# SamsungLabs/fcaf3d

Hardware: AMD Instinct MI355X
Metric: scenes/sec fwd+bwd, ScanNet 100k-pt 2cm voxels, 1/2/4/8 MI355X (higher is better)
Workload: dtype f32

## Files before the change

### fcaf3d_amd/csrc/conv.hip

```cpp
#include "fc_common.h"
#include "../../include/fcaf3d_hip.h"
#ifdef FC_TRACE
__device__ unsigned long long* g_trace_buf_lds;
__device__ int g_trace_cap_lds;
extern "C" int fc_debug_trace_lds(unsigned long long* buf, int cap) {
  FC_HIP(hipMemcpyToSymbol(HIP_SYMBOL(g_trace_buf_lds), &buf, sizeof(buf)));
  FC_HIP(hipMemcpyToSymbol(HIP_SYMBOL(g_trace_cap_lds), &cap, sizeof(cap)));
  return FC_OK;
}
#define TR_BUF g_trace_buf_lds
#define TR_CAP g_trace_cap_lds
#endif
#include "fc_trace.h"

typedef float f32x16 __attribute__((ext_vector_type(16)));
typedef float f32x2 __attribute__((ext_vector_type(2)));
typedef float f32x4 __attribute__((ext_vector_type(4)));

__device__ __attribute__((aligned(16))) float g_zero_row[64];

__device__ int g_fc_prio;
extern "C" int fc_debug_set_prio(int mode) {
  FC_HIP(hipMemcpyToSymbol(HIP_SYMBOL(g_fc_prio), &mode, sizeof(mode)));
  return FC_OK;
}

static int g_bf16_fast = 0;
extern "C" int fc_set_bf16_fast(int on) {
  g_bf16_fast = on ? 1 : 0;
  return FC_OK;
}

static int g_split_mode = 2;
static inline int split_mode() { return g_bf16_fast ? 0 : g_split_mode; }
extern "C" int fc_set_split_mode(int mode) {
  if (mode != 0 && mode != 2) return FC_EINVAL;
  g_split_mode = mode;
  return FC_OK;
}
extern "C" int fc_get_split_mode(void) { return split_mode(); }
static int g_h3r = 1;
extern "C" int fc_debug_set_h3r(int mode) {
  if (mode < 0 || mode > 2) return FC_EINVAL;
  g_h3r = mode;
  return FC_OK;
}

#include <mutex>
#include "conv_tile.h"
#include "conv_f32.h"
#include "wgrad_f32.h"
#include "conv_stem.h"
#include "conv_x6.h"
#include "wgrad_x6.h"
#include "conv_h3r.h"
#include "conv_route.h"
static inline RouteEnv route_env() { return {split_mode(), g_bf16_fast, g_h3r}; }

__global__ __launch_bounds__(256) void k_amax(const f32x4* __restrict__ x, int64_t n4, const float* __restrict__ tail, int ntail,
                                              unsigned* __restrict__ slot) {
  __shared__ unsigned wm[4];
  __shared__ int last_s;
  unsigned m = 0u;
  const int64_t stride = (int64_t)gridDim.x * 256;
  for (int64_t i = (int64_t)blockIdx.x * 256 + threadIdx.x; i < n4; i += 4 * stride) {
    f32x4 v[4];
#pragma unroll
    for (int q = 0; q < 4; ++q) v[q] = i + q * stride < n4 ? x[i + q * stride] : f32x4{0.f, 0.f, 0.f, 0.f};
#pragma unroll
    for (int q = 0; q < 4; ++q)
#pragma unroll
      for (int j = 0; j < 4; ++j) { const unsigned u = __float_as_uint(v[q][j]) & 0x7fffffffu; m = (u > m && u < 0x7f800000u) ? u : m; }
  }
  if (blockIdx.x == 0 && (int)threadIdx.x < ntail) { const unsigned u = __float_as_uint(tail[threadIdx.x]) & 0x7fffffffu; m = (u > m && u < 0x7f800000u) ? u : m; }
#pragma unroll
  for (int off = 32; off > 0; off >>= 1) { const unsigned o = (unsigned)__shfl_xor((int)m, off, 64); m = o > m ? o : m; }
  if ((threadIdx.x & 63) == 0) wm[threadIdx.x >> 6] = m;
  __syncthreads();
  if (threadIdx.x == 0) {
    unsigned b = wm[0];
    for (int w = 1; w < 4; ++w) b = wm[w] > b ? wm[w] : b;
    if (b > __hip_atomic_load(&slot[1], __ATOMIC_RELAXED, __HIP_MEMORY_SCOPE_AGENT)) atomicMax(&slot[1], b);
    __threadfence();
    last_s = atomicAdd(&slot[2], 1u) == gridDim.x - 1;
    if (last_s) {
      __threadfence();
      slot[0] = atomicExch(&slot[1], 0u);
      slot[2] = 0u;
    }
  }
}

constexpr int AMAX_RING = 2048;
static unsigned* g_amax_ring[16] = {};
static unsigned g_amax_next[16] = {};
static std::mutex g_amax_ring_mu;
static int amax_ring_slot(unsigned** slot) {
  int dev = 0;
  FC_HIP(hipGetDevice(&dev));
  if (dev < 0 || dev >= 16) return FC_EINVAL;
  std::lock_guard<std::mutex> lock(g_amax_ring_mu);
  if (!g_amax_ring[dev]) {
    FC_HIP(hipMalloc((void**)&g_amax_ring[dev], (size_t)AMAX_RING * FC_AMAX_SLOT_BYTES));
    FC_HIP(hipMemset(g_amax_ring[dev], 0, (size_t)AMAX_RING * FC_AMAX_SLOT_BYTES));
  }
  const unsigned i = __atomic_fetch_add(&g_amax_next[dev], 1u, __ATOMIC_RELAXED) % AMAX_RING;
  *slot = g_amax_ring[dev] + (size_t)i * (FC_AMAX_SLOT_BYTES / 4);
  return FC_OK;
}
static int amax_launch(const float* x, int64_t n, unsigned* slot, hipStream_t stream) {
// ... 145 lines not shown
#pragma unroll
      for (int u = 0; u < 9; ++u) {
        j[u] = k0 + u < K ? pos[(int64_t)(k0 + u) * n_out + o] : -1;
        j2[u] = (two && k0 + u < K) ? pos[(int64_t)(k0 + u) * n_out + o2] : -1;
      }
      f32x4 v[9], v2[9];
#pragma unroll
      for (int u = 0; u < 9; ++u) {
        const float* src = j[u] >= 0 ? part + ((int64_t)(k0 + u) * n_out + j[u]) * Cout + c : g_zero_row + lane * 4;
        const float* src2 = j2[u] >= 0 ? part + ((int64_t)(k0 + u) * n_out + j2[u]) * Cout + c : g_zero_row + lane * 4;
        v[u] = *reinterpret_cast<const f32x4*>(src);
        v2[u] = *reinterpret_cast<const f32x4*>(src2);
      }
#pragma unroll
      for (int u = 0; u < 9; ++u) {
        if (j[u] >= 0) a += v[u];
        if (j2[u] >= 0) b += v2[u];
      }
    }
    *reinterpret_cast<f32x4*>(out + o * Cout + c) = a;
    stat_accumulate(p, epi, a, o * Cout + c, a1, a2);
    if (two) {
      *reinterpret_cast<f32x4*>(out + o2 * Cout + c) = b;
      stat_accumulate(p, epi, b, o2 * Cout + c, a1, a2);
    }
  }
  stat_block_reduce(a1, a2, epi.stats, Cout, sm);
}

static_assert(STEM_CIN == 3 && STEM_COUT == 64 && BK == 32, "conv_route.h spells these shapes out");

struct ConvArgs {
  const float *in, *W; const int *nbr, *out_index, *cnt; float* dst;
  int64_t n_rows; int K, Cin, Cout; X6Epi epi; hipStream_t stream;
};
#define FC_LAUNCH(...) __VA_ARGS__<<<grid, 256, 0, a.stream>>>(a.in, a.W, a.nbr, a.out_index, a.cnt, a.dst, a.n_rows, a.K, a.Cin, a.Cout)
#define FC_LAUNCH_EPI(...) __VA_ARGS__<<<grid, 256, 0, a.stream>>>(a.in, a.W, a.nbr, a.out_index, a.cnt, a.dst, a.n_rows, a.K, a.Cin, a.Cout, a.epi)

template <int BM, int BN, int WM>
static void launch_conv_fp32(const ConvRoute& r, const ConvArgs& a, dim3 grid) {
#define FC_LAUNCH_MFMA(KERNEL)                                                                                              \
  do { if (r.wsrc == FC_WSRC_FP32_T) FC_LAUNCH(KERNEL<BM, BN, 32, true, WM, true>); else if (a.nbr) FC_LAUNCH(KERNEL<BM, BN, 32, true, WM>); \
       else FC_LAUNCH(KERNEL<BM, BN, 32, false, WM>); } while (0)
  if (r.family == FC_FAM_MFMA) FC_LAUNCH_MFMA(k_conv_mfma);
  if constexpr (BM >= 128) {
    if (r.family == FC_FAM_MFMA_P) FC_LAUNCH_MFMA(k_conv_mfma_p);
    if (r.family == FC_FAM_GLDS) { if (a.nbr) FC_LAUNCH(k_conv_glds<BM, BN, true, WM>); else FC_LAUNCH(k_conv_glds<BM, BN, false, WM>); }
  }
#undef FC_LAUNCH_MFMA
}

template <int BM, int BN, int WM>
static void launch_conv_x6(const ConvRoute& r, const ConvArgs& a, dim3 grid) {
  if (r.family == FC_FAM_H3R) {
    if constexpr (BM == 128) {
      if (r.buf) FC_LAUNCH_EPI(k_conv_h3r<BN, true, true>);
      else if (a.nbr) FC_LAUNCH_EPI(k_conv_h3r<BN, true, false>);
      else FC_LAUNCH_EPI(k_conv_h3r<BN, false, false>);
    }
  } else if (r.wsrc == FC_WSRC_FP32_T) FC_LAUNCH_EPI(k_conv_x6<BM, BN, true, WM, 1>);
  else if (r.wsrc == FC_WSRC_FP32) { if (a.nbr) FC_LAUNCH_EPI(k_conv_x6<BM, BN, true, WM, 0>); else FC_LAUNCH_EPI(k_conv_x6<BM, BN, false, WM, 0>); }
  else if (r.mode == FC_MODE_BF16 || r.buf) {
    if constexpr (BM == 128) {
      if (r.mode == FC_MODE_BF16) { if (a.nbr) FC_LAUNCH_EPI(k_conv_x6<128, BN, true, 2, 2, 1>); else FC_LAUNCH_EPI(k_conv_x6<128, BN, false, 2, 2, 1>); }
      else if (r.mode == FC_MODE_H3) FC_LAUNCH_EPI(k_conv_x6<128, BN, true, 2, 2, 2, true>);
      else FC_LAUNCH_EPI(k_conv_x6<128, BN, true, 2, 2, 0, true>);
    }
  } else if (r.mode == FC_MODE_H3) { if (a.nbr) FC_LAUNCH_EPI(k_conv_x6<BM, BN, true, WM, 2, 2>); else FC_LAUNCH_EPI(k_conv_x6<BM, BN, false, WM, 2, 2>); }
  else { if (a.nbr) FC_LAUNCH_EPI(k_conv_x6<BM, BN, true, WM, 2>); else FC_LAUNCH_EPI(k_conv_x6<BM, BN, false, WM, 2>); }
}

static int launch_conv(const ConvRoute& r, const ConvArgs& a) {
  const dim3 grid(r.grid[0], r.grid[1], r.grid[2]);
  if (r.family == FC_FAM_STEM) {
    const size_t smem = (size_t)(STEM_ROWS * STEM_FWD_LDA + 96 * 64) * sizeof(float);
    k_stem_fwd<<<(unsigned)fc_cdiv(a.n_rows, STEM_ROWS), 256, smem, a.stream>>>(a.in, a.W, a.nbr, a.dst, nullptr, a.n_rows, a.K);
  } else if (r.family == FC_FAM_FMA) {
    k_conv_fma<<<(unsigned)fc_cdiv(a.n_rows * a.Cout, 256), 256, 0, a.stream>>>(a.in, a.W, a.nbr, a.dst, a.n_rows, a.K, a.Cin, a.Cout, r.wsrc == FC_WSRC_FP32_T ? 1 : 0);
  } else {
#define FC_TILE(BM, BN, WM) do { if (r.family >= FC_FAM_X6) launch_conv_x6<BM, BN, WM>(r, a, grid); else launch_conv_fp32<BM, BN, WM>(r, a, grid); } while (0)
    if (r.bm == 256) FC_TILE(256, 64, 4);
    else if (r.bm == 128 && r.bn == 128) FC_TILE(128, 128, 2);
    else if (r.bm == 128) FC_TILE(128, 64, 2);
    else if (r.bn == 128) launch_conv_fp32<64, 128, 2>(r, a, grid);
    else launch_conv_fp32<64, 64, 2>(r, a, grid);
#undef FC_TILE
  }
  FC_CHECK_LAUNCH();
  return FC_OK;
}
#undef FC_LAUNCH
#undef FC_LAUNCH_EPI

extern "C" {

int fc_conv_fwd_route(int64_t n_in, int64_t n_out, int K, int Cin, int Cout, int flags, int table_kind, int64_t live_tiles, int* out) {
  if (!out || n_in < 0 || n_out < 0 || K < 1 || Cin < 1 || Cout < 1) return FC_EINVAL;
  const ConvRoute r = conv_route({n_in, n_out, K, Cin, Cout}, flags, table_kind, live_tiles, route_env());
  const int f[16] = {r.family, r.bm, r.bn, r.wm, r.S, r.wsrc, r.mode, r.buf, r.epi, (int)r.grid[0], (int)r.grid[1], (int)r.grid[2]};
  for (int i = 0; i < 16; ++i) out[i] = f[i];
  return r.family == FC_FAM_INVALID ? FC_EINVAL : FC_OK;
}

int64_t fc_conv_fwd_ws_bytes(int64_t n_out, int K, int Cin, int Cout, int flags) {
  const ConvRoute r = conv_route({n_out, n_out, K, Cin, Cout}, flags, FC_TABLE_DENSE, 0, route_env());
  return r.S > 1 ? (int64_t)r.S * n_out * Cout * (int64_t)sizeof(float) : 0;
}

int64_t fc_conv_fwd_pairs_ws_bytes(int64_t n_out, int K, int Cout) {
  return (int64_t)K * n_out * Cout * (int64_t)sizeof(float);
}

int64_t fc_conv_stats_blocks(int64_t n_out, int K, int Cin, int Cout, int flags, int pairs) {
  if (n_out < 1) return 0;
  const ConvRoute r = conv_route({n_out, n_out, K, Cin, Cout}, flags, pairs ? FC_TABLE_PAIRS : FC_TABLE_DENSE, 0, route_env());
  if (r.epi == FC_EPI_NONE) return 0;
  return r.epi == FC_EPI_SUM ? fc_cdiv(n_out, fc_stat_rb(n_out)) : fc_cdiv(n_out, r.bm);
}

static int conv_impl(const float* in, const float* W, const int* nbr, const int* out_index, const int* cnt, const int* pos, float* out,
                     int64_t n_in, int64_t n_out, int K, int Cin, int Cout, int64_t live_tiles, int flags, void* ws, int64_t ws_bytes,
                     hipStream_t stream, const X6Epi* epi) {
  AmaxHintScope hint_scope;
  if (n_in < 0 || n_out < 0 || K < 1 || Cin < 1 || Cout < 1) return FC_EINVAL;
  if (n_out == 0 && !cnt) return epi ? FC_EINVAL : FC_OK;
  if (out_index && !nbr) return FC_EINVAL;
  const int table = cnt ? FC_TABLE_PAIRS : out_index ? FC_TABLE_SORTED : nbr ? FC_TABLE_DENSE : FC_TABLE_NONE;
  const ConvRoute r = conv_route({n_in, n_out, K, Cin, Cout}, flags, table | (epi ? FC_TABLE_STATS : 0), live_tiles, route_env());
  if (r.family == FC_FAM_INVALID) return FC_EINVAL;
  if (n_out == 0) return FC_OK;
  ConvArgs a = {in, W, nbr, out_index, cnt, out, n_out, K, Cin, Cout, {}, stream};
  if (r.family == FC_FAM_STEM || r.family == FC_FAM_FMA) return launch_conv(r, a);
  const bool parts = cnt || r.S > 1;
  if (parts && ws_bytes < (int64_t)r.S * n_out * Cout * (int64_t)sizeof(float)) return FC_EWS;
  if (parts) a.dst = (float*)ws;
  if (epi && r.epi == FC_EPI_KERNEL) a.epi = *epi;
  int rc = FC_OK;
  if (r.mode == FC_MODE_H3) rc = operand_amax(in, n_in * (int64_t)Cin, 0, stream, &a.epi.amax_in);
  if (rc == FC_OK) rc = launch_conv(r, a);
  if (rc != FC_OK || !parts) return rc;
  const int rb = fc_stat_rb(n_out);
  const dim3 sgrid((unsigned)fc_cdiv(n_out, rb), Cout / 64);
  if (cnt && epi) k_sum_pairs_stats<<<sgrid, 256, 0, stream>>>(a.dst, pos, out, n_out, K, Cout, rb, *epi);
  else if (cnt) k_sum_pairs<<<(unsigned)fc_cdiv(n_out * (Cout / 4), 256), 256, 0, stream>>>(a.dst, pos, out, n_out, K, Cout);
  else if (epi) k_sum_parts_stats<<<sgrid, 256, 0, stream>>>(a.dst, out, n_out, Cout, r.S, rb, *epi);
  else k_sum_parts<<<(unsigned)fc_cdiv(n_out * Cout / 4, 256), 256, 0, stream>>>(a.dst, out, n_out * Cout / 4, r.S);
  FC_CHECK_LAUNCH();
  return FC_OK;
}

static int conv_pairs_impl(const float* in, const float* W, const int* pair_in, const int* pair_cnt, const int* pair_pos, float* out,
                           int64_t n_in, int64_t n_out, int K, int Cin, int Cout, int64_t live_tiles, int flags, void* ws,
// ... 323 lines not shown
```

### fcaf3d_amd/csrc/conv_route.h

```cpp
#ifndef FC_CONV_ROUTE_H
#define FC_CONV_ROUTE_H
#include "fc_common.h"
#include "../../include/fcaf3d_hip.h"

struct RouteEnv { int split_mode, bf16_fast, h3r; };
struct ConvShape { int64_t n_in, n_out; int K, Cin, Cout; };

struct ConvRoute {
  int family;
  int bm, bn, wm;
  int S;
  int wsrc, mode, buf, epi;
  unsigned grid[3];
};
struct WgradRoute {
  int family;
  int bm, bn, ko, bkr;
  int table, mode, S;
  int64_t rps;
  int wbuf;
  unsigned grid_y;
};

static inline int flag_bm(int flags) { return (flags >> FC_CONV_BM_SHIFT) & FC_CONV_TILE_MASK; }
static inline int flag_bn(int flags) { return (flags >> FC_CONV_BN_SHIFT) & FC_CONV_TILE_MASK; }
static inline int flag_s(int flags) { return (flags >> FC_CONV_S_SHIFT) & FC_CONV_S_MASK; }
static inline bool below_2gb(uint64_t bytes) { return bytes < (1ull << 31) - 4096u; }

static inline bool stem_shape(int K, int Cin, int Cout, int flags) { return !(flags & FC_CONV_FMA) && Cin == 3 && Cout == 64 && K <= 27; }

static inline int offset_split(int64_t tiles, int K) {
  if (K <= 1 || tiles >= 384) return 1;
  return (int)(1024 / tiles < K ? 1024 / tiles : K);
}

static inline ConvRoute conv_route(const ConvShape& s, int flags, int table, int64_t live_tiles, const RouteEnv& env) {
  const bool stats = (table & FC_TABLE_STATS) != 0;
  table &= ~FC_TABLE_STATS;
  const bool pairs = table == FC_TABLE_PAIRS, gather = table != FC_TABLE_NONE, split = (flags & FC_CONV_SPLIT) != 0;
  const bool image = split && (flags & FC_CONV_IMAGE);
  const bool wt = (flags & FC_CONV_WT) && !image;
  const int64_t n = s.n_out > 0 ? s.n_out : 1;
  const int K = s.K, Cin = s.Cin, Cout = s.Cout;
  ConvRoute r = {};
  r.family = FC_FAM_INVALID;
  r.wsrc = image ? FC_WSRC_IMAGE : wt ? FC_WSRC_FP32_T : FC_WSRC_FP32;
  if (!gather && (K != 1 || s.n_in != s.n_out)) return r;
  if ((flags & FC_CONV_WT) && !gather) return r;
  const bool mfma = Cin % 32 == 0 && Cout % 64 == 0 && (pairs || (!(flags & FC_CONV_FMA) && K <= 32));
  if (pairs && !mfma) return r;
  if (stats && !(mfma && split)) return r;
  r.bn = (Cout % 128 == 0) ? 128 : 64;
  if (pairs) {
    if (flag_bn(flags) == 1) r.bn = 64;
    r.bm = 128;
    r.S = K;
  } else {
    r.bm = (n > 64 && fc_cdiv(n, 128) * (Cout / r.bn) >= 4) ? 128 : 64;
    if (Cout == 64 && fc_cdiv(n, 256) >= 1024 && !split) r.bm = 256;
    const int fbm = flag_bm(flags), fbn = flag_bn(flags);
    if (fbm) r.bm = fbm == 1 ? 64 : (fbm == 2 ? 128 : 256);
    if (fbn && (Cout % (fbn == 1 ? 64 : 128) == 0)) r.bn = fbn == 1 ? 64 : 128;
    if (r.bm == 256) r.bn = 64;
    if (split && mfma && r.bm == 64) r.bm = 128;
    r.S = mfma ? offset_split(fc_cdiv(n, r.bm) * (Cout / r.bn), K) : 1;
    if (flag_s(flags)) r.S = flag_s(flags) > K ? K : flag_s(flags);
  }
  r.wm = r.bm == 256 ? 4 : 2;
  if (stem_shape(K, Cin, Cout, flags) && !(flags & FC_CONV_WT) && table == FC_TABLE_DENSE) { r.family = FC_FAM_STEM; return r; }
  if (!mfma && table != FC_TABLE_SORTED && !(flags & FC_CONV_IMAGE)) r.family = FC_FAM_FMA;
  if (!mfma) return r;
  r.grid[0] = (unsigned)fc_cdiv(n, r.bm), r.grid[1] = (unsigned)(Cout / r.bn), r.grid[2] = (unsigned)r.S;
  if (pairs && live_tiles > 0) r.grid[0] = (unsigned)live_tiles, r.grid[2] = 1;
  if (split) {
    r.family = FC_FAM_X6;
    r.mode = !image ? FC_MODE_SIX : (env.bf16_fast && r.bm == 128) ? FC_MODE_BF16 : env.split_mode == 2 ? FC_MODE_H3 : FC_MODE_SIX;
    if (r.mode == FC_MODE_H3 && r.bm == 128 && (env.h3r == 2 || (env.h3r == 1 && r.bn == 128))) r.family = FC_FAM_H3R;
    r.buf = image && gather && r.bm == 128 && r.mode != FC_MODE_BF16 && !(flags & FC_CONV_FLAT) &&
            below_2gb((uint64_t)s.n_in * (uint64_t)Cin * 4u) && below_2gb((uint64_t)K * (uint64_t)s.n_out * 4u);
    r.epi = (pairs || r.S > 1) ? FC_EPI_SUM : FC_EPI_KERNEL;
    return r;
  }
  const int64_t wgs = (int64_t)r.grid[0] * r.grid[1] * r.grid[2];
  r.mode = FC_MODE_FP32;
  if (flags & FC_CONV_GLDS) r.family = FC_FAM_GLDS;
  else if (flags & FC_CONV_PIPE_ON) r.family = FC_FAM_MFMA_P;
  else if ((flags & FC_CONV_PIPE_OFF) || (pairs && live_tiles <= 0)) r.family = FC_FAM_MFMA;
  else if (wgs >= 1536 || wgs <= 768) r.family = FC_FAM_MFMA_P;
  else r.family = (r.grid[2] > 1 && !(flags & FC_CONV_GLDS_OFF)) ? FC_FAM_GLDS : FC_FAM_MFMA;
  if (r.family == FC_FAM_GLDS && wt) r.family = FC_FAM_MFMA;
  if (r.bm == 64) r.family = FC_FAM_MFMA;
  return r;
}

#define WGRAD_KO 3

static inline WgradRoute wgrad_route(const ConvShape& s, int flags, int table, const RouteEnv& env) {
  const int64_t n = s.n_out > 0 ? s.n_out : 1;
  const int K = s.K, Cin = s.Cin, Cout = s.Cout, fbm = flag_bm(flags), fbn = flag_bn(flags);
  const bool dense = table == FC_TABLE_DENSE, pairs = table == FC_TABLE_PAIRS, split = (flags & FC_CONV_SPLIT) != 0;
  if (pairs) flags &= ~FC_CONV_WGRAD_DEEP;
  WgradRoute r = {};
  r.family = FC_WFAM_INVALID;
  r.table = table, r.ko = 1, r.bkr = 32, r.mode = FC_MODE_FP32;
  if (table == FC_TABLE_SORTED || (table == FC_TABLE_NONE && (K != 1 || s.n_in != s.n_out))) return r;
  const bool mfma = !(flags & FC_CONV_FMA) && Cin % 64 == 0 && Cout % 64 == 0;
  if (pairs && !mfma) return r;
  if (stem_shape(K, Cin, Cout, flags)) {
    r.family = dense ? FC_WFAM_STEM : FC_WFAM_FMA;
    r.rps = 1024, r.S = (int)fc_cdiv(n, 1024), r.grid_y = dense ? 1 : (unsigned)K;
    return r;
  }
  const bool multi = dense && mfma && !(flags & FC_CONV_WGRAD_MULTI_OFF) && K % WGRAD_KO == 0 && n >= 4096 &&
                     (!(flags & FC_CONV_WGRAD_MULTI_FIRST) || (Cin == 64 && n >= 32768));
  const bool x6t = mfma && split && (multi || !dense);
  const int wide = (Cout % 128 == 0) ? 128 : 64;
  r.bm = 64;
  r.bn = wide;
  if (fbm == 2 && Cin % 128 == 0) r.bm = 128;
  if (fbn == 1) r.bn = 64;
  if (fbn == 2 && Cout % 128 == 0) r.bn = 128;
  if (split && !dense && Cin % 128 == 0) r.bm = 128;
  int64_t sp = 1728 / (mfma ? (int64_t)K * (Cin / r.bm) * (Cout / r.bn) : (int64_t)K);
  if (multi) {
    constexpr int round_wide = 256, round_narrow = 512;
    sp = (wide == 128 ? round_wide : round_narrow) / ((int64_t)(K / WGRAD_KO) * (Cin / 64) * (Cout / wide));
  }
  const int64_t max_by_rows = fc_cdiv(n, mfma ? 512 : 2048);
  sp = sp > max_by_rows ? max_by_rows : sp;
  sp = sp > 256 ? 256 : sp < 1 ? 1 : sp;
  if (flag_s(flags)) sp = flag_s(flags);
  r.rps = fc_align(fc_cdiv(n, sp), 64);
  r.S = (int)fc_cdiv(n, r.rps);
// ... 23 lines not shown
```

### include/fcaf3d_hip.h

```cpp
#ifndef FCAF3D_HIP_H
#define FCAF3D_HIP_H
#include <stdint.h>

#ifndef __HIP_PLATFORM_AMD__
typedef struct ihipStream_t* hipStream_t;
#endif

#ifdef __cplusplus
extern "C" {
#endif

#define FC_ABI_VERSION 19
#ifndef FC_AMAX_SLOT_BYTES
#define FC_AMAX_SLOT_BYTES 2048
#endif
int fc_abi_version(void);


int fc_voxelize(const float* points, int64_t n, int pt_stride, int batch_idx, float voxel_size, float feat_div,
                int nfeat, int* coords, float* feats, hipStream_t stream);

int fc_augment_voxelize(const float* points, int64_t n_src, int pt_stride, const int* sample_idx, int64_t n_out,
                        const float* xform_host, int batch_idx, float voxel_size, float feat_div, int nfeat, int* coords,
                        float* feats, float* points_out, hipStream_t stream);
// ... 83 lines not shown

int64_t fc_conv_fwd_ws_bytes(int64_t n_out, int K, int Cin, int Cout, int flags);
int fc_conv_fwd(const float* in, const float* W, const int* nbr, const int* out_index, float* out, int64_t n_in,
                int64_t n_out, int K, int Cin, int Cout, int flags, void* ws, int64_t ws_bytes, hipStream_t stream);

int64_t fc_conv_fwd_pairs_ws_bytes(int64_t n_out, int K, int Cout);
int fc_conv_fwd_pairs(const float* in, const float* W, const int* pair_in, const int* pair_cnt, const int* pair_pos,
                      float* out, int64_t n_in, int64_t n_out, int K, int Cin, int Cout, int flags, void* ws,
                      int64_t ws_bytes, hipStream_t stream);

int fc_conv_fwd_pairs_tiles(const float* in, const float* W, const int* pair_in, const int* pair_cnt, const int* pair_pos,
                            float* out, int64_t n_in, int64_t n_out, int K, int Cin, int Cout, int64_t live_tiles, int flags,
                            void* ws, int64_t ws_bytes, hipStream_t stream);

int64_t fc_conv_stats_blocks(int64_t n_out, int K, int Cin, int Cout, int flags, int pairs);
int fc_conv_fwd_stats(const float* in, const float* W, const int* nbr, const int* out_index, float* out, int64_t n_in,
                      int64_t n_out, int K, int Cin, int Cout, int flags, void* ws, int64_t ws_bytes, float* stats,
                      hipStream_t stream);
int fc_conv_fwd_pairs_tiles_stats(const float* in, const float* W, const int* pair_in, const int* pair_cnt, const int* pair_pos,
                                  float* out, int64_t n_in, int64_t n_out, int K, int Cin, int Cout, int64_t live_tiles, int flags,
                                  void* ws, int64_t ws_bytes, float* stats, hipStream_t stream);
int fc_conv_fwd_bn_bwd_stats(const float* in, const float* W, const int* nbr, const int* out_index, float* out, int64_t n_in,
                             int64_t n_out, int K, int Cin, int Cout, int flags, void* ws, int64_t ws_bytes, float* stats,
                             const float* bn_x, const float* mean, const float* var, const float* gamma, const float* beta, float eps,
                             int act, const float* add, const float* bn_y, hipStream_t stream);
int fc_conv_fwd_pairs_tiles_bn_bwd_stats(const float* in, const float* W, const int* pair_in, const int* pair_cnt, const int* pair_pos,
                                         float* out, int64_t n_in, int64_t n_out, int K, int Cin, int Cout, int64_t live_tiles, int flags,
                                         void* ws, int64_t ws_bytes, float* stats, const float* bn_x, const float* mean,
                                         const float* var, const float* gamma, const float* beta, float eps, int act,
                                         const float* add, const float* bn_y, hipStream_t stream);

int64_t fc_conv_wgrad_ws_bytes(int64_t n_out, int K, int Cin, int Cout, int flags);
int fc_conv_wgrad(const float* in, const float* gout, const int* nbr, const int* row_index, float* gW, int64_t n_in,
                  int64_t n_out, int K, int Cin, int Cout, int flags, void* ws, int64_t ws_bytes, hipStream_t stream);
int fc_conv_wgrad_pairs(const float* in, const float* gout, const int* pair_in, const int* pair_out, const int* pair_cnt,
                        float* gW, int64_t n_in, int64_t n_out, int K, int Cin, int Cout, int flags, void* ws,
                        int64_t ws_bytes, hipStream_t stream);

int fc_stem_conv_fwd(const float* in, const float* W, const int* nbr, float* out, float* col, int64_t n_in, int64_t n_out,
                     int K, hipStream_t stream);
int64_t fc_stem_conv_wgrad_ws_bytes(int64_t n_out, int K);
int fc_stem_conv_wgrad(const float* col, const float* gout, float* gW, int64_t n_out, int K, void* ws, int64_t ws_bytes,
                       hipStream_t stream);

int fc_transpose_weight(const float* W, float* Wt, int K, int Cin, int Cout, hipStream_t stream);

enum { FC_TABLE_NONE, FC_TABLE_DENSE, FC_TABLE_SORTED, FC_TABLE_PAIRS, FC_TABLE_STATS = 8 };
enum { FC_FAM_INVALID, FC_FAM_STEM, FC_FAM_FMA, FC_FAM_MFMA, FC_FAM_MFMA_P, FC_FAM_GLDS, FC_FAM_X6, FC_FAM_H3R };
enum { FC_WFAM_INVALID, FC_WFAM_STEM, FC_WFAM_FMA, FC_WFAM_MFMA, FC_WFAM_MFMA_P, FC_WFAM_MULTI, FC_WFAM_X6T };
enum { FC_WSRC_FP32, FC_WSRC_FP32_T, FC_WSRC_IMAGE };
enum { FC_MODE_FP32, FC_MODE_SIX, FC_MODE_BF16, FC_MODE_H3 };
enum { FC_EPI_NONE, FC_EPI_KERNEL, FC_EPI_SUM };
enum { FC_ROUTE_FAMILY, FC_ROUTE_BM, FC_ROUTE_BN, FC_ROUTE_WM, FC_ROUTE_S, FC_ROUTE_WSRC, FC_ROUTE_MODE, FC_ROUTE_BUF, FC_ROUTE_EPI,
       FC_ROUTE_GRID_X, FC_ROUTE_GRID_Y, FC_ROUTE_GRID_Z };
enum { FC_WROUTE_FAMILY, FC_WROUTE_BM, FC_WROUTE_BN, FC_WROUTE_KO, FC_WROUTE_BKR, FC_WROUTE_TABLE, FC_WROUTE_MODE, FC_WROUTE_S,
       FC_WROUTE_RPS, FC_WROUTE_WBUF, FC_WROUTE_GRID_Y };
int fc_conv_fwd_route(int64_t n_in, int64_t n_out, int K, int Cin, int Cout, int flags, int table_kind, int64_t live_tiles,
                      int* out);
int fc_conv_wgrad_route(int64_t n_in, int64_t n_out, int K, int Cin, int Cout, int flags, int table_kind, int* out);


int64_t fc_col_stats_ws_bytes(int64_t n, int C, int nseg);
int fc_col_stats(const float* x, const int* seg, int seg_stride, int64_t n, int C, int nseg, float* mean, float* var,
                 float* cnt, void* ws, int64_t ws_bytes, hipStream_t stream);

int fc_seg_col_sums(const float* x, const int* seg, int seg_stride, int64_t n, int C, int nseg, float* out, void* ws,
                    int64_t ws_bytes, hipStream_t stream);
int fc_bn_running_update(const float* mean, const float* var, const float* cnt, float momentum, int C, float* running_mean,
                         float* running_var, long long* num_batches_tracked, hipStream_t stream);

int fc_norm_act_fwd(const float* x, const int* seg, int seg_stride, int64_t n, int C, const float* mean, const float* var,
                    float eps, const float* gamma, const float* beta, const float* residual, int act, float* y,
                    hipStream_t stream);
int64_t fc_norm_act_bwd_ws_bytes(int64_t n, int C, int nseg);
int fc_norm_act_bwd(const float* x, const float* y, const float* gy, const int* seg, int seg_stride, int64_t n, int C,
                    int nseg, const float* mean, const float* var, const float* cnt, float eps, const float* gamma,
                    const float* beta, int act, float* gx, float* gres, float* sums, void* ws, int64_t ws_bytes,
                    hipStream_t stream);

int64_t fc_bn_stats_ws_bytes(int64_t n, int C);
int fc_bn_stats_train(const float* x, int64_t n, int C, float momentum, float* mean, float* var, float* cnt,
                      float* running_mean, float* running_var, long long* num_batches_tracked, void* ws,
                      int64_t ws_bytes, hipStream_t stream);
int64_t fc_bn_small_ws_bytes(int C);
int fc_bn_act_train_fwd(const float* x, int64_t n, int C, float eps, const float* gamma, const float* beta,
                        const float* residual, int act, float momentum, float* y, float* mean, float* var, float* cnt,
                        float* running_mean, float* running_var, long long* num_batches_tracked, void* ws,
                        int64_t ws_bytes, hipStream_t stream);
int fc_bn_act_train_bwd(const float* x, const float* y, const float* gy, int64_t n, int C, const float* mean,
                        const float* var, float eps, const float* gamma, const float* beta, int act, float* gx, float* gres,
                        float* sums, void* ws, int64_t ws_bytes, hipStream_t stream);

int64_t fc_bn_train_ws_bytes(int64_t n, int C);
int fc_bn_train_fwd(const float* x, int64_t n, int C, float eps, const float* gamma, const float* beta, const float* residual,
                    int act, float momentum, float* y, float* mean, float* var, float* cnt, float* running_mean,
                    float* running_var, long long* num_batches_tracked, const float* part, int64_t nb_part, int groups,
                    int64_t small_elems, void* ws, int64_t ws_bytes, hipStream_t stream);
int fc_bn_train_bwd(const float* x, const float* y, const float* gy, const float* gy2, int64_t n, int C, const float* mean,
                    const float* var, const float* cnt, float eps, const float* gamma, const float* beta, int act, float* gx,
                    float* gres, float* sums, const float* part, int64_t nb_part, int64_t small_elems, void* ws, int64_t ws_bytes,
                    hipStream_t stream);

enum { FC_NFORM_TRAIN, FC_NFORM_SMALL, FC_NFORM_SEG };
enum { FC_NSTATS_INVALID, FC_NSTATS_PROLOGUE, FC_NSTATS_PARTIAL_SMALL, FC_NSTATS_PARTIAL, FC_NSTATS_TABLE };
enum { FC_NAPPLY_NONE, FC_NAPPLY_BN1, FC_NAPPLY_BN2, FC_NAPPLY_ROWS };
enum { FC_NAMAX_NONE, FC_NAMAX_FOLDED, FC_NAMAX_PASS };
enum { FC_NRED_INVALID, FC_NRED_TABLE, FC_NRED_PARTIAL, FC_NRED_NONE };
// ... 103 lines not shown
#define FC_MERGE_WITH_YAW 2
#define FC_MERGE_XF_FLIP_H (1ull << 32)
#define FC_MERGE_XF_FLIP_V (1ull << 33)
int64_t fc_merge_sorted_segments_ws_bytes(int nseg_out, int max_total);
int fc_merge_sorted_segments(const int64_t* desc, int nseg_out, int K, const int* counts_dev, const int* keep, int keep_stride,
                             const int64_t* ord, int ord_stride, const float* scores, int score_stride, const float* boxes,
                             int flags, int max_total, int cap, float* out_boxes, float* out_scores, int* out_src,
                             int* out_count, int stride_out, void* ws, int64_t ws_bytes, hipStream_t stream);


#define FC_VOTE_ROTATED 1
#define FC_VOTE_WITH_YAW 2
int fc_vote_boxes(const float* boxes, const float* scores, const int* counts_dev, int nseg, int stride, int max_count,
                  const int* keep, const int* keep_counts_dev, int keep_stride, int max_keep, float vote_thr, int flags,
                  float* out_boxes, int* out_members, hipStream_t stream);


#define FC_EVAL_DET_BOTTOM 1
int64_t fc_eval_match_ws_bytes(int64_t n_det, int64_t n_gt, int n_thr);
int fc_eval_match(const float* det_boxes, int det_dim , const float* det_scores, const int64_t* det_labels,
                  const float* gt_boxes , const int* gt_labels,
                  const int64_t* seg , int n_scenes,
                  int64_t n_det, int64_t n_gt, const double* thr , int n_thr, int flags,
                  float* best_iou, int* best_gt, unsigned char* tp_bits, void* ws, int64_t ws_bytes, hipStream_t stream);


int64_t fc_grad_norm_ws_bytes(int64_t n);
int fc_grad_norm(const float* g, int64_t n, float max_norm, float* out, void* ws, int64_t ws_bytes, hipStream_t stream);
int fc_adamw_step(float* p, const float* g, float* m, float* v, int64_t n, float lr, float beta1, float beta2, float eps,
                  float weight_decay, float bias_correction1, float bias_correction2, const float* norm_and_clip,
                  hipStream_t stream);

#define FC_ADAMW_MAX_RUNS 1024
int64_t fc_adamw_groups_table_bytes(int R);
int fc_adamw_groups_pack(const int64_t* begin, const float* lr_mult, const float* decay_mult, int R, int64_t n, void* out,
                         int64_t out_bytes);
int fc_adamw_step_groups(float* p, const float* g, float* m, float* v, int64_t n, float lr, float beta1, float beta2, float eps,
                         float weight_decay, float bias_correction1, float bias_correction2, const float* norm_and_clip,
                         const void* table_dev, int R, hipStream_t stream);

int fc_adamw_ema_step(float* p, const float* g, float* m, float* v, float* ema, int64_t n, float lr, float beta1, float beta2,
                      float eps, float weight_decay, float bias_correction1, float bias_correction2, const float* norm_and_clip,
                      const void* table_dev, int R, float ema_mu, float ema_keep, hipStream_t stream);
int fc_swap_f32(float* a, float* b, int64_t n, hipStream_t stream);

int fc_set_bf16_fast(int on);

int fc_set_split_mode(int mode);
int fc_get_split_mode(void);
int fc_amax(const float* x, int64_t n, unsigned* slot, hipStream_t stream);
int fc_conv_amax_hint(const unsigned* amax_in, const unsigned* amax_gout);
int fc_amax_out_hint(unsigned* amax_word);
int fc_debug_set_h3r(int mode);


int fc_exec_op_words(void);
int64_t fc_exec_probe_read(float* ms, int64_t* meta, int64_t cap);
int fc_exec_map_words(void);
int fc_exec(const int64_t* ops, int64_t op_begin, int64_t op_end, const int64_t* addr, const int64_t* dims, const int64_t* maps,
            const int64_t* streams, const int64_t* ws, const int64_t* ws_bytes, int64_t* ws_need, const int64_t* cfg);

#ifdef __cplusplus
}
#endif
#endif
```

Measured before the change: 537.6.

## Add persistent LDS-resident-weight kernel for dense 1x1 split-precision convolutions

Adds a persistent kernel for non-gather (dense) H3 split-precision convolutions. It loads the whole weight column block into LDS once per workgroup, then loops over row tiles with a capped grid. Row loads are software-pipelined: the next slab is prefetched while MFMAs run on the current one. It fuses BN-stat partial sums into the epilogue, which can pair waves to chain the sums. Weights are no longer re-fetched per tile. The trade-off is larger dynamic LDS, lower occupancy, and a new routing path that a debug flag can switch off.

```diff
diff --git a/fcaf3d_amd/csrc/conv.hip b/fcaf3d_amd/csrc/conv.hip
--- a/fcaf3d_amd/csrc/conv.hip
+++ b/fcaf3d_amd/csrc/conv.hip
@@ -45,6 +45,12 @@
   g_h3r = mode;
   return FC_OK;
 }
+static int g_dense = 1;
+extern "C" int fc_debug_set_dense(int on) {
+  if (on < 0 || on > 1) return FC_EINVAL;
+  g_dense = on;
+  return FC_OK;
+}
 
 #include <mutex>
 #include "conv_tile.h"
@@ -54,8 +60,9 @@
 #include "conv_x6.h"
 #include "wgrad_x6.h"
 #include "conv_h3r.h"
+#include "conv_dense.h"
 #include "conv_route.h"
-static inline RouteEnv route_env() { return {split_mode(), g_bf16_fast, g_h3r}; }
+static inline RouteEnv route_env() { return {split_mode(), g_bf16_fast, g_h3r, g_dense}; }
 
 __global__ __launch_bounds__(256) void k_amax(const f32x4* __restrict__ x, int64_t n4, const float* __restrict__ tail, int ntail,
                                               unsigned* __restrict__ slot) {
@@ -307,7 +314,14 @@
 
 template <int BM, int BN, int WM>
 static void launch_conv_x6(const ConvRoute& r, const ConvArgs& a, dim3 grid) {
-  if (r.family == FC_FAM_H3R) {
+  if (r.stream) {
+    if constexpr (BM == 128) {
+      const size_t smem = (size_t)a.Cin * BN * 4 + (size_t)(4 * BN * 2 + 2 * (BN / 32) * 2 * 64 + 4 * BN) * sizeof(float);
+#define FC_LAUNCH_DENSE(PAIRS) k_conv_dense<BN, PAIRS><<<grid, 256, smem, a.stream>>>(a.in, a.W, a.dst, a.n_rows, a.Cin, a.Cout, a.epi)
+      if (r.family == FC_FAM_H3R) FC_LAUNCH_DENSE(false); else FC_LAUNCH_DENSE(true);
+#undef FC_LAUNCH_DENSE
+    }
+  } else if (r.family == FC_FAM_H3R) {
     if constexpr (BM == 128) {
       if (r.buf) FC_LAUNCH_EPI(k_conv_h3r<BN, true, true>);
       else if (a.nbr) FC_LAUNCH_EPI(k_conv_h3r<BN, true, false>);
@@ -352,7 +366,7 @@
 int fc_conv_fwd_route(int64_t n_in, int64_t n_out, int K, int Cin, int Cout, int flags, int table_kind, int64_t live_tiles, int* out) {
   if (!out || n_in < 0 || n_out < 0 || K < 1 || Cin < 1 || Cout < 1) return FC_EINVAL;
   const ConvRoute r = conv_route({n_in, n_out, K, Cin, Cout}, flags, table_kind, live_tiles, route_env());
-  const int f[16] = {r.family, r.bm, r.bn, r.wm, r.S, r.wsrc, r.mode, r.buf, r.epi, (int)r.grid[0], (int)r.grid[1], (int)r.grid[2]};
+  const int f[16] = {r.family, r.bm, r.bn, r.wm, r.S, r.wsrc, r.mode, r.buf, r.epi, (int)r.grid[0], (int)r.grid[1], (int)r.grid[2], r.stream};
   for (int i = 0; i < 16; ++i) out[i] = f[i];
   return r.family == FC_FAM_INVALID ? FC_EINVAL : FC_OK;
 }
diff --git a/fcaf3d_amd/csrc/conv_dense.h b/fcaf3d_amd/csrc/conv_dense.h
--- /dev/null
+++ b/fcaf3d_amd/csrc/conv_dense.h
@@ -0,0 +1,237 @@
+#pragma once
+
+template <int BN, bool PAIRS>
+__global__ __launch_bounds__(256, BN == 64 ? 4 : 3) void k_conv_dense(
+    const float* __restrict__ in, const float* __restrict__ W, float* __restrict__ out, int64_t n_out, int Cin, int Cout, X6Epi epi) {
+  constexpr int BM = 128;
+  constexpr int TN = BN / 32;
+  constexpr int NG = BN / 64;
+  constexpr int GU = 2 * 64 * 4;
+  constexpr int BU = 3 * BN / 64;
+  constexpr int UB = BN == 128 ? 2 : 4;
+  extern __shared__ u32x4 dense_sm[];
+  float* __restrict__ stats = epi.stats;
+
+  const int tid = threadIdx.x, lane = tid & 63;
+  const int wave = __builtin_amdgcn_readfirstlane(tid >> 6);
+  const int r = lane & 31, h = lane >> 5;
+  const int n0 = blockIdx.y * BN;
+  const int nslab = Cin / 32, ngrp = Cout / 64;
+  const int64_t tiles = (n_out + BM - 1) / BM;
+  u32x4* Bs = dense_sm;
+  float* red = reinterpret_cast<float*>(dense_sm + nslab * NG * GU);
+  float* chain = red + 4 * BN * 2;
+  float* par = chain + 2 * TN * 2 * 64;
+
+  const float h3_sa = h3_scale(fc_amax_read(epi.amax_in));
+  const float h3_inv = h3_unscale(h3_sa, h3_scale(fc_amax_read(reinterpret_cast<const unsigned*>(W) + X6_IMG_AMAX_WORD)));
+
+  {
+    const u32x4* img = reinterpret_cast<const u32x4*>(W);
+    for (int s = 0; s < nslab; ++s) {
+      const u32x4* src = img + ((int64_t)s * ngrp + n0 / 64) * X6_GROUP_U16 + tid;
+#pragma unroll
+      for (int i = 0; i < BU; ++i)
+        if (i % 3 != 2) Bs[s * (NG * GU) + (i / 3) * GU + (i % 3) * 256 + tid] = src[256 * i];
+    }
+  }
+  const bool bwd = stats && epi.bn_x != nullptr;
+  const bool from_y = bwd && epi.bn_y != nullptr && epi.act != 0;
+  if (bwd && tid < BN) {
+    const int col = n0 + tid;
+    par[0 * BN + tid] = epi.mean[col];
+    par[1 * BN + tid] = 1.f / sqrtf(epi.var[col] + epi.eps);
+    par[2 * BN + tid] = epi.gamma ? epi.gamma[col] : 1.f;
+    par[3 * BN + tid] = epi.beta ? epi.beta[col] : 0.f;
+  }
+  const int swz = (r >> 2) & 3;
+  int b_slot[2];
+#pragma unroll
+  for (int b = 0; b < 2; ++b) b_slot[b] = r * 4 + ((2 * b + h) ^ swz);
+  const int lrow = wave * 32 + r;
+
+  f32x4 av[4];
+  auto load_stage = [&](int64_t t, int s) {
+    const int64_t row = t * BM + lrow;
+    const bool live = row < n_out;
+    const float* rowp = live ? in + row * Cin + s * 32 + 8 * h : g_zero_row;
+#pragma unroll
+    for (int q = 0; q < 4; ++q) av[q] = *reinterpret_cast<const f32x4*>(rowp + (live ? 16 * (q >> 1) + 4 * (q & 1) : 4 * q));
+  };
+  u32x4 fa[2][2];
+  auto split_rows = [&]() {
+#pragma unroll
+    for (int b = 0; b < 2; ++b) {
+      unsigned p0[4], p1[4];
+#pragma unroll
+      for (int q = 0; q < 2; ++q) {
+        h3_split2s(av[2 * b + q][0], av[2 * b + q][1], h3_sa, p0[2 * q], p1[2 * q]);
+        h3_split2s(av[2 * b + q][2], av[2 * b + q][3], h3_sa, p0[2 * q + 1], p1[2 * q + 1]);
+      }
+      fa[b][0] = u32x4{p0[0], p0[1], p0[2], p0[3]};
+      fa[b][1] = u32x4{p1[0], p1[1], p1[2], p1[3]};
+    }
+  };
+
+  int64_t t = blockIdx.x;
+  if (t < tiles) load_stage(t, 0);
+  __syncthreads();
+  if (t < tiles) split_rows();
+  for (; t < tiles; t += gridDim.x) {
+    const int64_t m0 = t * BM;
+    f32x16 acc[TN];
+#pragma unroll
+    for (int j = 0; j < TN; ++j)
+#pragma unroll
+      for (int e = 0; e < 16; ++e) acc[j][e] = 0.f;
+    for (int s = 0; s < nslab; ++s) {
+      if (s + 1 < nslab) load_stage(t, s + 1); else load_stage(t + gridDim.x, 0);
+      __builtin_amdgcn_sched_barrier(0);
+      const u32x4* B = Bs + s * (NG * GU);
+#pragma unroll
+      for (int b = 0; b < 2; ++b) {
+#pragma unroll
+        for (int pb = 1; pb >= 0; --pb) {
+          u32x4 fb[TN];
+#pragma unroll
+          for (int j = 0; j < TN; ++j) fb[j] = B[(j >> 1) * GU + pb * 256 + (j & 1) * 32 * 4 + b_slot[b]];
+#pragma unroll
+          for (int pa = 1 - pb; pa >= 0; --pa)
+#pragma unroll
+            for (int j = 0; j < TN; ++j) acc[j] = H3_MFMA(fa[b][pa], fb[j], acc[j]);
+        }
+      }
+      split_rows();
+    }
+#pragma unroll
+    for (int j = 0; j < TN; ++j)
+#pragma unroll
+      for (int e = 0; e < 16; ++e) acc[j][e] *= h3_inv;
+
+    const int64_t rb = m0 + wave * 32 + 4 * h;
+    const int lim = (int)(n_out - rb < 32 ? n_out - rb : 32);
+    const int64_t at0 = rb * Cout + n0 + 2 * r;
+    if (stats) {
+      float s1[TN], s2[TN];
+#pragma unroll
+      for (int j = 0; j < TN; ++j) { s1[j] = 0.f; s2[j] = 0.f; }
+      float mu[TN], is[TN], ga[TN], be[TN];
+#pragma unroll
+      for (int j = 0; j < TN; ++j) {
+        const int cl = (j >> 1) * 64 + 2 * r + (j & 1);
+        mu[j] = 0.f; is[j] = 1.f; ga[j] = 1.f; be[j] = 0.f;
+        if (bwd) { mu[j] = par[0 * BN + cl]; is[j] = par[1 * BN + cl]; ga[j] = par[2 * BN + cl]; be[j] = par[3 * BN + cl]; }
+      }
+      auto sum_rows = [&]() {
+#pragma unroll
+        for (int e0 = 0; e0 < 16; e0 += UB) {
+          float xv[UB][TN], av2[UB][TN], yv[UB][TN];
+#pragma unroll
+          for (int u = 0; u < UB; ++u) {
+            const int eo = ((e0 + u) & 3) + 8 * ((e0 + u) >> 2);
+#pragma unroll
+            for (int j = 0; j < TN; ++j) { xv[u][j] = 0.f; av2[u][j] = 0.f; yv[u][j] = 0.f; }
+            if (bwd && eo < lim) {
+#pragma unroll
+              for (int g = 0; g < NG; ++g) {
+                const int64_t at = at0 + eo * Cout + g * 64;
+                const f32x2 x2 = *reinterpret_cast<const f32x2*>(epi.bn_x + at);
+                xv[u][2 * g] = x2[0]; xv[u][2 * g + 1] = x2[1];
+                if (epi.add) { const f32x2 a2 = *reinterpret_cast<const f32x2*>(epi.add + at); av2[u][2 * g] = a2[0]; av2[u][2 * g + 1] = a2[1]; }
+                if (from_y) { const f32x2 y2 = *reinterpret_cast<const f32x2*>(epi.bn_y + at); yv[u][2 * g] = y2[0]; yv[u][2 * g + 1] = y2[1]; }
+              }
+            }
+          }
+#pragma unroll
+          for (int u = 0; u < UB; ++u) {
+            if (bwd && ((e0 + u) & 3) + 8 * ((e0 + u) >> 2) >= lim) continue;
+#pragma unroll
+            for (int j = 0; j < TN; ++j) {
+              float t1, t2;
+              x6_epi_terms(bwd, bwd ? av2[u][j] + acc[j][e0 + u] : acc[j][e0 + u], xv[u][j], mu[j], is[j], ga[j], be[j], epi.act, from_y,
+                           yv[u][j], t1, t2);
+              s1[j] += t1;
+              s2[j] += t2;
+            }
+          }
+        }
+      };
+      if (PAIRS) {
+        const int pair = wave >> 1;
+        if (!(wave & 1)) {
+          sum_rows();
+#pragma unroll
+          for (int j = 0; j < TN; ++j) {
+            chain[((pair * TN + j) * 2 + 0) * 64 + lane] = s1[j];
+            chain[((pair * TN + j) * 2 + 1) * 64 + lane] = s2[j];
+          }
+        }
+        __syncthreads();
+        if (wave & 1) {
+#pragma unroll
+          for (int j = 0; j < TN; ++j) {
+            s1[j] = chain[((pair * TN + j) * 2 + 0) * 64 + lane];
+            s2[j] = chain[((pair * TN + j) * 2 + 1) * 64 + lane];
+          }
+          sum_rows();
+#pragma unroll
+          for (int j = 0; j < TN; ++j) {
+            s1[j] += __shfl_xor(s1[j], 32, 64);
+            s2[j] += __shfl_xor(s2[j], 32, 64);
+          }
+          if (h == 0) {
+#pragma unroll
+            for (int j = 0; j < TN; ++j) {
+              const int cl = (j >> 1) * 64 + 2 * r + (j & 1);
+              red[(pair * BN + cl) * 2 + 0] = s1[j];
+              red[(pair * BN + cl) * 2 + 1] = s2[j];
+            }
+          }
+        }
+        __syncthreads();
+        if (tid < BN) {
+          float a = 0.f, b = 0.f;
+#pragma unroll
+          for (int w = 0; w < 2; ++w) { a += red[(w * BN + tid) * 2 + 0]; b += red[(w * BN + tid) * 2 + 1]; }
+          stats[((int64_t)t * 2 + 0) * Cout + n0 + tid] = a;
+          stats[((int64_t)t * 2 + 1) * Cout + n0 + tid] = b;
+        }
+      } else {
+        sum_rows();
+#pragma unroll
+        for (int j = 0; j < TN; ++j) {
+          s1[j] += __shfl_xor(s1[j], 32, 64);
+          s2[j] += __shfl_xor(s2[j], 32, 64);
+        }
+        __syncthreads();
+        if (h == 0) {
+#pragma unroll
+          for (int j = 0; j < TN; ++j) {
+            const int cl = (j >> 1) * 64 + 2 * r + (j & 1);
+            red[(wave * BN + cl) * 2 + 0] = s1[j];
+            red[(wave * BN + cl) * 2 + 1] = s2[j];
+          }
+        }
+        __syncthreads();
+        if (tid < BN) {
+          float a = 0.f, b = 0.f;
+#pragma unroll
+          for (int w = 0; w < 4; ++w) { a += red[(w * BN + tid) * 2 + 0]; b += red[(w * BN + tid) * 2 + 1]; }
+          stats[((int64_t)t * 2 + 0) * Cout + n0 + tid] = a;
+          stats[((int64_t)t * 2 + 1) * Cout + n0 + tid] = b;
+        }
+      }
+    }
+#pragma unroll
+    for (int e = 0; e < 16; ++e) {
+      const int eo = (e & 3) + 8 * (e >> 2);
+      if (eo < lim) {
+#pragma unroll
+        for (int g = 0; g < NG; ++g) {
+          f32x2 v = {acc[2 * g][e], acc[2 * g + 1][e]};
+          *reinterpret_cast<f32x2*>(out + at0 + eo * Cout + g * 64) = v;
+        }
+      }
+    }
+  }
+}
diff --git a/fcaf3d_amd/csrc/conv_route.h b/fcaf3d_amd/csrc/conv_route.h
--- a/fcaf3d_amd/csrc/conv_route.h
+++ b/fcaf3d_amd/csrc/conv_route.h
@@ -3,7 +3,7 @@
 #include "fc_common.h"
 #include "../../include/fcaf3d_hip.h"
 
-struct RouteEnv { int split_mode, bf16_fast, h3r; };
+struct RouteEnv { int split_mode, bf16_fast, h3r, dense; };
 struct ConvShape { int64_t n_in, n_out; int K, Cin, Cout; };
 
 struct ConvRoute {
@@ -12,6 +12,7 @@
   int S;
   int wsrc, mode, buf, epi;
   unsigned grid[3];
+  int stream;
 };
 struct WgradRoute {
   int family;
@@ -33,6 +34,9 @@
   if (K <= 1 || tiles >= 384) return 1;
   return (int)(1024 / tiles < K ? 1024 / tiles : K);
 }
+
+#define DENSE_LDS_BYTES 32768
+#define DENSE_SLOTS 768
 
 static inline ConvRoute conv_route(const ConvShape& s, int flags, int table, int64_t live_tiles, const RouteEnv& env) {
   const bool stats = (table & FC_TABLE_STATS) != 0;
@@ -79,6 +83,13 @@
     r.buf = image && gather && r.bm == 128 && r.mode != FC_MODE_BF16 && !(flags & FC_CONV_FLAT) &&
             below_2gb((uint64_t)s.n_in * (uint64_t)Cin * 4u) && below_2gb((uint64_t)K * (uint64_t)s.n_out * 4u);
     r.epi = (pairs || r.S > 1) ? FC_EPI_SUM : FC_EPI_KERNEL;
+    if (!gather && env.dense && r.mode == FC_MODE_H3 && r.bm == 128 && Cin * 64 * 4 <= DENSE_LDS_BYTES) {
+      r.stream = 1;
+      r.bn = (r.bn == 128 && Cin * 128 * 4 <= DENSE_LDS_BYTES) ? 128 : 64;
+      const int64_t tiles = fc_cdiv(n, 128), groups = Cout / r.bn;
+      const int64_t slots = DENSE_SLOTS / groups > 0 ? DENSE_SLOTS / groups : 1;
+      r.grid[0] = (unsigned)fc_cdiv(tiles, fc_cdiv(tiles, slots)), r.grid[1] = (unsigned)groups, r.grid[2] = 1;
+    }
     return r;
   }
   const int64_t wgs = (int64_t)r.grid[0] * r.grid[1] * r.grid[2];
diff --git a/include/fcaf3d_hip.h b/include/fcaf3d_hip.h
--- a/include/fcaf3d_hip.h
+++ b/include/fcaf3d_hip.h
@@ -159,7 +159,7 @@
 enum { FC_MODE_FP32, FC_MODE_SIX, FC_MODE_BF16, FC_MODE_H3 };
 enum { FC_EPI_NONE, FC_EPI_KERNEL, FC_EPI_SUM };
 enum { FC_ROUTE_FAMILY, FC_ROUTE_BM, FC_ROUTE_BN, FC_ROUTE_WM, FC_ROUTE_S, FC_ROUTE_WSRC, FC_ROUTE_MODE, FC_ROUTE_BUF, FC_ROUTE_EPI,
-       FC_ROUTE_GRID_X, FC_ROUTE_GRID_Y, FC_ROUTE_GRID_Z };
+       FC_ROUTE_GRID_X, FC_ROUTE_GRID_Y, FC_ROUTE_GRID_Z, FC_ROUTE_STREAM };
 enum { FC_WROUTE_FAMILY, FC_WROUTE_BM, FC_WROUTE_BN, FC_WROUTE_KO, FC_WROUTE_BKR, FC_WROUTE_TABLE, FC_WROUTE_MODE, FC_WROUTE_S,
        FC_WROUTE_RPS, FC_WROUTE_WBUF, FC_WROUTE_GRID_Y };
 int fc_conv_fwd_route(int64_t n_in, int64_t n_out, int K, int Cin, int Cout, int flags, int table_kind, int64_t live_tiles,
@@ -369,6 +369,7 @@
 int fc_conv_amax_hint(const unsigned* amax_in, const unsigned* amax_gout);
 int fc_amax_out_hint(unsigned* amax_word);
 int fc_debug_set_h3r(int mode);
+int fc_debug_set_dense(int on);
 
 
 int fc_exec_op_words(void);
```

New measurement: 539.3 (median of 4 runs). About the same (+0.3%).
